# aikiriao/LINNE

Measured on NVIDIA B200. Metric: encode+decode MSamples/s over the -m 0..7 sweep, higher is better.
Workload: dtype int32+f64

## Files before the change

linne_b200/csrc/lnb_analyze_v3.cuh:

```cuda
#pragma once
#include "lnb_common.cuh"
#include "lnb_encode_core.cuh"

#define LNB_A3_THREADS  256
#define LNB_A3_WARPS    8
#define LNB_A3_MAX_NA   10240
#define LNB_A3_FRONT    160
#define LNB_A3_BACK     176
#define LNB_A3_PART     24
#define LNB_A3_ITEMS    64
#define LNB_A3_MIRROR   (LNB_MAX_PARAMS + 8)

__host__ __device__ inline uint32_t lnb_a3_array_doubles(uint32_t na_max)
{
    if (na_max < 4096u) na_max = 4096u;
    return LNB_A3_FRONT + na_max / 8u * 9u + LNB_A3_BACK;
}
__host__ __device__ inline size_t lnb_a3_smem_doubles(uint32_t na_max)
{
    return (size_t)2 * lnb_a3_array_doubles(na_max)
         + (size_t)LNB_MAX_LEVELS * LNB_MAX_PARAMS
         + (size_t)LNB_MAX_LEVELS * 256
         + (size_t)LNB_A3_ITEMS * LNB_A3_PART
         + (size_t)3 * LNB_A3_MIRROR
         + 128;
}

struct LnbA3Ctx {
    double *A, *B;
    double *cand, *acorr, *part, *lev0, *misc;
    uint32_t na, ng;
};

struct LnbA3Team {
    uint32_t tid, nthr, warp, nwarps, bar;
    __device__ __forceinline__ void sync() const
    {
        if (bar == 0u) __syncthreads();
        else asm volatile("bar.sync %0, %1;" :: "r"(bar), "r"(nthr) : "memory");
    }
};

__device__ __forceinline__ void lnb_a3_window(const LnbA3Ctx &cx, const LnbA3Team &tm, uint32_t m, double scale)
{
    const uint32_t mg = m >> 3;
    for (uint32_t G = tm.tid; G < cx.ng; G += tm.nthr) {
        const uint32_t pos0 = (G % mg) * 8u;
        const double *src = cx.A + G * 9u;
        double *dst = cx.B + G * 9u;
        const uint32_t back0 = m - 1u - pos0;
        const double a0 = (double)pos0, b0 = (double)back0;
        if (pos0 + 7u <= back0 - 7u || pos0 >= back0) {
            const bool rising = pos0 < back0;
#pragma unroll
            for (uint32_t e = 0; e < 8u; e++) {
                const double a = a0 + (double)e, b = b0 - (double)e;
                const double w = rising ? __dmul_rn(__dmul_rn(scale, a), b) : __dmul_rn(__dmul_rn(scale, b), a);
                dst[e] = __dmul_rn(src[e], w);
            }
        } else {
#pragma unroll
            for (uint32_t e = 0; e < 8u; e++) {
                const double a = a0 + (double)e, b = b0 - (double)e;
                const double q = (a < b) ? a : b, r = (a < b) ? b : a;
                dst[e] = __dmul_rn(src[e], __dmul_rn(__dmul_rn(scale, q), r));
            }
        }
    }
}

template <int L, bool MASK>
__device__ __forceinline__ void lnb_a3_tile(const double *Bg, uint32_t qoff, int32_t lim, double (&acc)[L])
{
    double s[8], wv[L + 7];
#pragma unroll
    for (int o = 0; o < 8; o++) s[o] = Bg[o];
#pragma unroll
    for (int t = 0; t < L + 7; t++) {
        const double v = (!MASK || t < lim) ? Bg[qoff + t + (t >> 3)] : 0.0;
        wv[t] = v;
    }
#pragma unroll
    for (int o = 0; o < 8; o++)
#pragma unroll
        for (int k = 0; k < L; k++) acc[k] = fma(s[o], wv[o + k], acc[k]);
}

template <int L>
__device__ __forceinline__ void lnb_a3_autocorr_item(const LnbA3Ctx &cx, uint32_t u, uint32_t q, uint32_t m, bool last_unit,
                                                     uint32_t g_lo, uint32_t g_hi, double *out )
{
    const uint32_t lane = threadIdx.x & 31u;
    const uint32_t mg = m >> 3;
    double acc[L];
#pragma unroll
    for (int k = 0; k < L; k++) acc[k] = 0.0;
    const double *Bu = cx.B + (size_t)u * mg * 9u;
    const uint32_t qoff = 18u * q;
    for (uint32_t g0 = g_lo; g0 < g_hi; g0 += 32u) {
        const uint32_t g = g0 + lane;
        const bool active = g < g_hi;
        const uint32_t gg = active ? g : g_lo;
        const int32_t lim = (int32_t)m - (int32_t)(8u * gg + 16u * q);
        const bool need_mask = !last_unit && lim < L + 7;
        if (__any_sync(0xffffffffu, need_mask)) {
            double tmp[L];
#pragma unroll
            for (int k = 0; k < L; k++) tmp[k] = 0.0;
            lnb_a3_tile<L, true>(Bu + gg * 9u, qoff, last_unit ? (int32_t)(L + 7) : lim, tmp);
            if (active) {
#pragma unroll
                for (int k = 0; k < L; k++) acc[k] += tmp[k];
            }
        } else if (active) {
            lnb_a3_tile<L, false>(Bu + gg * 9u, qoff, 0, acc);
        }
    }
    constexpr int N = (L >= 16) ? 16 : (L >= 8) ? 8 : (L >= 4) ? 4 : 2;
    constexpr int LOGN = (N == 16) ? 4 : (N == 8) ? 3 : (N == 4) ? 2 : 1;
    {
        int cnt = N;
#pragma unroll
        for (int off = 16; off > 0; off >>= 1) {
            if (cnt > 1) {
                const bool upper = (lane & (uint32_t)off) != 0u;
                const int half = cnt / 2;
#pragma unroll
                for (int k = 0; k < N / 2; k++) {
                    if (k < half) {
                        const double send = upper ? acc[k] : acc[k + half];
                        const double keep = upper ? acc[k + half] : acc[k];
                        acc[k] = keep + __shfl_xor_sync(0xffffffffu, send, off);
                    }
                }
                cnt = half;
            } else {
                acc[0] += __shfl_xor_sync(0xffffffffu, acc[0], off);
            }
        }
        if ((lane & ((1u << (5 - LOGN)) - 1u)) == 0u) out[lane >> (5 - LOGN)] = acc[0];
    }
    if (L > N) {
        double v = acc[L - 1];
#pragma unroll
        for (int off = 16; off > 0; off >>= 1) v += __shfl_xor_sync(0xffffffffu, v, off);
        if (lane == 0) out[L - 1] = v;
    }
}

__device__ void lnb_a3_autocorr(const LnbA3Ctx &cx, const LnbA3Team &tm, uint32_t U, uint32_t p, double *acorr_lvl)
{
    const uint32_t m = cx.na / U, mg = m >> 3;
    const uint32_t nq = (p >= 16u) ? p / 16u : 1u;
    const uint32_t tasks = U * nq;
    uint32_t S = 1u;
    if ((tasks % tm.nwarps) != 0u && tasks < 4u * tm.nwarps) S = (3u * tm.nwarps + tasks - 1u) / tasks;
    if (tasks * S > LNB_A3_ITEMS) S = LNB_A3_ITEMS / tasks;
    const uint32_t items = tasks * S;
    const uint32_t per = (mg + S - 1u) / S;
    for (uint32_t wi = tm.warp; wi < items; wi += tm.nwarps) {
        const uint32_t task = wi / S, split = wi % S;
        const uint32_t u = task / nq, q = task % nq;
        const uint32_t g_lo = split * per, g_hi = (g_lo + per < mg) ? g_lo + per : mg;
        const bool last_unit = (u + 1u == U);
        double *out = (S == 1u) ? acorr_lvl + u * (p + 1u) + 16u * q : cx.part + wi * LNB_A3_PART;
        if (p >= 16u) {
            if (q + 1u < nq) lnb_a3_autocorr_item<16>(cx, u, q, m, last_unit, g_lo, g_hi, out);
            else             lnb_a3_autocorr_item<17>(cx, u, q, m, last_unit, g_lo, g_hi, out);
        } else if (p == 8u)  lnb_a3_autocorr_item<9>(cx, u, q, m, last_unit, g_lo, g_hi, out);
        else if (p == 4u)    lnb_a3_autocorr_item<5>(cx, u, q, m, last_unit, g_lo, g_hi, out);
        else if (p == 2u)    lnb_a3_autocorr_item<3>(cx, u, q, m, last_unit, g_lo, g_hi, out);
        else                 lnb_a3_autocorr_item<2>(cx, u, q, m, last_unit, g_lo, g_hi, out);
    }
    if (S > 1u) {
        tm.sync();
        const uint32_t L_last = (p >= 16u) ? 17u : p + 1u;
        for (uint32_t i = tm.tid; i < tasks * 17u; i += tm.nthr) {
            const uint32_t task = i / 17u, k = i % 17u;
            const uint32_t u = task / nq, q = task % nq;
            const uint32_t Lq = (q + 1u == nq) ? L_last : 16u;
            if (k >= Lq) continue;
            double v = 0.0;
            for (uint32_t sp = 0; sp < S; sp++) v += cx.part[(task * S + sp) * LNB_A3_PART + k];
            acorr_lvl[u * (p + 1u) + 16u * q + k] = v;
        }
    }
}

__device__ __forceinline__ double lnb_a3_rcp(double x)
{
    float seed;
    asm("rcp.approx.ftz.f32 %0, %1;" : "=f"(seed) : "f"(__double2float_rn(x)));
    double y = (double)seed;
    y = fma(y, fma(-x, y, 1.0), y);
    y = fma(y, fma(-x, y, 1.0), y);
    y = fma(y, fma(-x, y, 1.0), y);
    return y;
}

__device__ void lnb_a3_levinson_warp(const double *r_in, uint32_t p, double lambda, double *scr, double *out_w)
{
    const uint32_t lane = threadIdx.x & 31u;
    const double r0 = __dmul_rn(r_in[0], __dadd_rn(1.0, lambda));
    if (fabs(r0) < (double)FLT_EPSILON) {
        for (uint32_t i = lane; i < p; i += 32u) out_w[i] = 0.0;
        return;
    }
    double *cur = scr, *nxt = scr + LNB_A3_MIRROR, *gam = scr + 2 * LNB_A3_MIRROR;
    double B[5];
#pragma unroll
    for (int s = 0; s < 5; s++) {
        const uint32_t i = lane + 32u * (uint32_t)s;
        const double ri = (i <= p) ? r_in[i] : 0.0;
        B[s] = (i == 0u) ? r0 : ri;
        if (i < LNB_A3_MIRROR) { cur[i] = ri; nxt[i] = 0.0; }
    }
    __syncwarp();
    double rinv = lnb_a3_rcp(r0);
    for (uint32_t m = 1; m <= p; m++) {
        const double gamma = -cur[1] * rinv;
        if (lane == 0) gam[m] = gamma;
        const uint32_t cnt = p - m;
        const uint32_t ns = (cnt >> 5) + 1u;
#pragma unroll
        for (int s = 0; s < 5; s++) {
            if ((uint32_t)s < ns) {
                const uint32_t i = lane + 32u * (uint32_t)s;
                if (i <= cnt) {
                    const double fs = cur[i + 1u];
                    const double b = B[s];
                    B[s] = fma(gamma, fs, b);
                    nxt[i] = fma(gamma, b, fs);
                }
            }
        }
        const double err = __shfl_sync(0xffffffffu, B[0], 0);
        rinv = lnb_a3_rcp(err);
        __syncwarp();
        double *t = cur; cur = nxt; nxt = t;
    }
    double a[5];
#pragma unroll
    for (int s = 0; s < 5; s++) {
        const uint32_t i = lane + 32u * (uint32_t)s;
        a[s] = (i == 0u) ? 1.0 : 0.0;
        if (i < LNB_A3_MIRROR) { cur[i] = a[s]; nxt[i] = a[s]; }
    }
    __syncwarp();
    for (uint32_t m = 1; m <= p; m++) {
        const double g = gam[m];
        const uint32_t ns = (m >> 5) + 1u;
#pragma unroll
        for (int s = 0; s < 5; s++) {
            if ((uint32_t)s < ns) {
                const uint32_t i = lane + 32u * (uint32_t)s;
                if (i >= 1u && i <= m) {
                    const double v = (i == m) ? g : fma(g, cur[m - i], a[s]);
                    a[s] = v;
                    nxt[i] = v;
                }
            }
        }
        __syncwarp();
        double *t = cur; cur = nxt; nxt = t;
    }
#pragma unroll
    for (int s = 0; s < 5; s++) {
        const uint32_t i = lane + 32u * (uint32_t)s;
        if (i >= 1u && i <= p) out_w[p - i] = a[s];
    }
    __syncwarp();
}

__device__ __forceinline__ void lnb_a3_fir8(const double *base, const double *w, const double (&prev)[8], double (&next)[8],
                                            double (&acc)[8])
{
#pragma unroll
    for (int k = 0; k < 8; k++) next[k] = base[7 + k + ((7 + k) >> 3)];
#pragma unroll
    for (int jj = 0; jj < 8; jj++) {
        const double wj = w[jj];
#pragma unroll
        for (int o = 0; o < 8; o++) {
            const int t = jj + o;
            acc[o] = fma(wj, (t < 7) ? prev[t + 1] : next[t - 7], acc[o]);
        }
    }
}

template <int MODE, int PS>
__device__ __forceinline__ double lnb_a3_fir(const LnbA3Ctx &cx, const LnbA3Team &tm, const double *X, double *Y, uint32_t p,
                                             uint32_t m, const double *cand_lvl)
{
    const uint32_t mg = m >> 3;
    double loss = 0.0;
    for (uint32_t G = tm.tid; G < cx.ng; G += tm.nthr) {
        const uint32_t u = G / mg;
        const double *w = cand_lvl + u * p;
        const double *Xg = X + G * 9u;
        double acc[8];
#pragma unroll
        for (int o = 0; o < 8; o++) acc[o] = (MODE == 0) ? Xg[o] : 0.0;
        if (PS == 0) {
            const double *base = Xg - (p >> 3) * 9u;
            double P[8], Q[8];
#pragma unroll
            for (int k = 0; k < 7; k++) P[k + 1] = base[k];
            uint32_t j0 = 0;
            for (; j0 + 16u <= p; j0 += 16u) {
                lnb_a3_fir8(base, w + j0, P, Q, acc);
                base += 9;
                lnb_a3_fir8(base, w + j0 + 8u, Q, P, acc);
                base += 9;
            }
            if (j0 < p) lnb_a3_fir8(base, w + j0, P, Q, acc);
        } else {
            double xw[PS + 7];
#pragma unroll
            for (int t = 0; t < PS + 7; t++) xw[t] = (t < PS) ? Xg[t - 1 - PS] : Xg[t - PS];
#pragma unroll
            for (int jj = 0; jj < PS; jj++) {
                const double wj = w[jj];
#pragma unroll
                for (int o = 0; o < 8; o++) acc[o] = fma(wj, xw[jj + o], acc[o]);
            }
        }
        if (MODE == 0) {
#pragma unroll
            for (int o = 0; o < 8; o++) if (!(G == 0u && o == 0)) loss += fabs(acc[o]);
        } else {
            double *Yg = Y + G * 9u;
#pragma unroll
            for (int o = 0; o < 8; o++) {
                const double y = Xg[o] + acc[o];
                Yg[o] = y;
                loss += fabs(y);
            }
        }
    }
    return loss;
}

template <int MODE>
__device__ double lnb_a3_fir_any(const LnbA3Ctx &cx, const LnbA3Team &tm, const double *X, double *Y, uint32_t p, uint32_t m,
                                 const double *cand_lvl)
{
    if (p >= 8u) return lnb_a3_fir<MODE, 0>(cx, tm, X, Y, p, m, cand_lvl);
    if (p == 4u) return lnb_a3_fir<MODE, 4>(cx, tm, X, Y, p, m, cand_lvl);
    if (p == 2u) return lnb_a3_fir<MODE, 2>(cx, tm, X, Y, p, m, cand_lvl);
    return lnb_a3_fir<MODE, 1>(cx, tm, X, Y, p, m, cand_lvl);
}

__device__ double lnb_a3_team_sum(const LnbA3Team &tm, double v, double *scratch )
{
#pragma unroll
    for (int off = 16; off > 0; off >>= 1) v += __shfl_xor_sync(0xffffffffu, v, off);
    tm.sync();
    if ((tm.tid & 31u) == 0) scratch[tm.warp] = v;
    tm.sync();
    double s = 0.0;
    for (uint32_t w = 0; w < tm.nwarps; w++) s += scratch[w];
    tm.sync();
    return s;
}
__device__ double lnb_a3_block_sum(double v, double *scratch)
{
    const LnbA3Team all = { threadIdx.x, LNB_A3_THREADS, threadIdx.x >> 5, LNB_A3_WARPS, 0u };
    return lnb_a3_team_sum(all, v, scratch);
}

__device__ void lnb_a3_level_losses(const LnbA3Ctx &cx, const LnbA3Team &tm, uint32_t P, uint32_t lv_first, uint32_t nlev)
{
    double *parts = cx.misc + 32;
    for (uint32_t lv = lv_first; lv < nlev; lv++) {
        const uint32_t U = 1u << lv, p = P / U;
        double v = lnb_a3_fir_any<0>(cx, tm, cx.A, (double *)0, p, cx.na / U, cx.cand + lv * LNB_MAX_PARAMS);
#pragma unroll
        for (int off = 16; off > 0; off >>= 1) v += __shfl_xor_sync(0xffffffffu, v, off);
        if ((tm.tid & 31u) == 0u) parts[tm.warp * LNB_MAX_LEVELS + lv] = v;
    }
    tm.sync();
    if (tm.tid >= lv_first && tm.tid < nlev) {
        double sum = 0.0;
        for (uint32_t w = 0; w < tm.nwarps; w++) sum += parts[w * LNB_MAX_LEVELS + tm.tid];
        cx.misc[tm.tid] = sum / (double)cx.na;
    }
}

__device__ void lnb_a3_solve_levels(const LnbA3Ctx &cx, const LnbA3Team &tm, uint32_t P, uint32_t lv_first, uint32_t nlev,
                                    double lambda, double *scratch)
{
    uint32_t thread_tasks = 0, warp_tasks = 0;
    for (uint32_t lv = lv_first; lv < nlev; lv++) { if ((P >> lv) <= 16u) thread_tasks += 1u << lv; else warp_tasks += 1u << lv; }
    for (uint32_t t = tm.tid; t < thread_tasks; t += tm.nthr) {
        uint32_t rest = t;
        for (uint32_t lv = lv_first; lv < nlev; lv++) {
            const uint32_t U = 1u << lv, p = P / U;
            if (p > 16u) continue;
            if (rest < U) {
                double r[17], a[18], coef[16];
                const double *src = cx.acorr + lv * 256 + rest * (p + 1u);
                for (uint32_t k = 0; k <= p; k++) r[k] = src[k];
                r[0] = __dmul_rn(r[0], __dadd_rn(1.0, lambda));
                lnb_levinson(r, p, a, coef, (double *)0);
                double *dst = cx.cand + lv * LNB_MAX_PARAMS + rest * p;
                for (uint32_t j = 0; j < p; j++) dst[j] = coef[p - 1u - j];
                break;
            }
            rest -= U;
        }
    }
    for (uint32_t t = tm.warp; t < warp_tasks; t += tm.nwarps) {
        uint32_t rest = t;
        for (uint32_t lv = lv_first; lv < nlev; lv++) {
            const uint32_t U = 1u << lv, p = P / U;
            if (p <= 16u) continue;
            if (rest < U) {
                lnb_a3_levinson_warp(cx.acorr + lv * 256 + rest * (p + 1u), p, lambda,
                                     scratch + tm.warp * 3 * LNB_A3_MIRROR, cx.cand + lv * LNB_MAX_PARAMS + rest * p);
                break;
            }
            rest -= U;
        }
    }
}

__device__ void lnb_a3_generic(const LnbEncodeBatch &b, uint32_t s, uint32_t bc, uint32_t blk_i, uint32_t na,
                               double lambda, uint32_t na_max, double *smem)
{
    const uint32_t c = threadIdx.x, warp = c >> 5;
    const uint32_t arr = lnb_a3_array_doubles(na_max);
    double *A = smem, *B = smem + arr;
    double *cand = smem + 2u * arr, *acorr = cand + LNB_MAX_LEVELS * LNB_MAX_PARAMS;
    double *misc = acorr + LNB_MAX_LEVELS * 256 + LNB_A3_ITEMS * LNB_A3_PART + 3 * LNB_A3_MIRROR;
    {
        const int32_t *src = b.work + (size_t)bc * b.cfg.work_stride;
        const double norm = ldexp(1.0, -(int)(b.cfg.bits_per_sample - 1u));
        for (uint32_t i = c; i < na; i += LNB_A3_THREADS) A[i] = (double)src[i] * norm;
    }
    __syncthreads();
    double final_loss = 0.0;
    for (uint32_t l = 0; l < b.cfg.num_layers; l++) {
        const uint32_t P = b.cfg.layer_params[l];
        for (uint32_t lv = 0; lv < LNB_MAX_LEVELS; lv++) {
            if (!lnb_level_valid(lv, P, na)) continue;
            const uint32_t U = 1u << lv, p = P / U, m = na / U;
            const double scale = b.welch[(size_t)blk_i * LNB_MAX_LEVELS + lv];
            for (uint32_t i = c; i < na; i += LNB_A3_THREADS)
                B[i] = lnb_mul_rn(A[i], lnb_welch_weight(scale, i % m, m));
            __syncthreads();
            for (uint32_t cell = c; cell < U * (p + 1u); cell += LNB_A3_THREADS) {
                const uint32_t lag = cell % (p + 1u);
                const double *xs = B + (size_t)(cell / (p + 1u)) * m;
                double sum = 0.0;
                for (uint32_t i = 0; i + lag < m; i++) sum = lnb_mac(xs[i], xs[i + lag], sum);
                acorr[lv * 256u + cell] = sum;
            }
            __syncthreads();
        }
        {
            uint32_t task = c, wt = warp;
            for (uint32_t lv = 0; lv < LNB_MAX_LEVELS; lv++) {
                if (!lnb_level_valid(lv, P, na)) continue;
                const uint32_t U = 1u << lv, p = P / U, m = na / U;
                if (p <= 16u) {
                    if (task < U) {
                        double r[17], a[18], coef[16];
                        const double *src = acorr + lv * 256u + task * (p + 1u);
                        for (uint32_t k = 0; k <= p; k++) r[k] = src[k];
                        r[0] = __dmul_rn(r[0], __dadd_rn(1.0, lambda));
                        if (m < p) { for (uint32_t k = 0; k < p; k++) coef[k] = 0.0; }
                        else lnb_levinson(r, p, a, coef, (double *)0);
                        double *dst = cand + lv * LNB_MAX_PARAMS + task * p;
                        for (uint32_t j = 0; j < p; j++) dst[j] = coef[p - 1u - j];
                        task = 0xFFFFFFFFu;
                    } else if (task != 0xFFFFFFFFu) task -= U;
                } else {
                    if (wt < U) {
                        double *dst = cand + lv * LNB_MAX_PARAMS + wt * p;
                        if (m < p) { for (uint32_t j = c & 31u; j < p; j += 32u) dst[j] = 0.0; }
                        else lnb_a3_levinson_warp(acorr + lv * 256u + wt * (p + 1u), p, lambda, B + warp * 3 * LNB_A3_MIRROR, dst);
                        wt = 0xFFFFFFFFu;
                    } else if (wt != 0xFFFFFFFFu) wt -= U;
                }
            }
        }
        __syncthreads();
        uint32_t best = 0;
        {
            double best_loss = (double)FLT_MAX;
            for (uint32_t lv = 0; lv < LNB_MAX_LEVELS; lv++) {
                if (!lnb_level_valid(lv, P, na)) continue;
                const uint32_t U = 1u << lv, p = P / U, m = na / U;
                double part = 0.0;
                for (uint32_t t = c; t < na; t += LNB_A3_THREADS)
                    if (t) part += fabs(lnb_residual_at(A, t, m, p, cand + lv * LNB_MAX_PARAMS, A[t]));
                const double loss = lnb_a3_block_sum(part, misc + 16) / (double)na;
                if (loss < best_loss) { best_loss = loss; best = lv; }
            }
        }
        if (c == 0) b.chosen_log2u[(size_t)s * LNB_MAX_LAYERS + l] = (uint8_t)best;
        {
            double *dst = b.chosen_w + ((size_t)s * LNB_MAX_LAYERS + l) * LNB_MAX_PARAMS;
            for (uint32_t k = c; k < P; k += LNB_A3_THREADS) dst[k] = cand[best * LNB_MAX_PARAMS + k];
        }
        {
            const uint32_t U = 1u << best, p = P / U, m = na / U;
            double part = 0.0;
            for (uint32_t t = c; t < na; t += LNB_A3_THREADS) {
                const double v = (t == 0u) ? A[0] : A[t] + lnb_residual_at(A, t, m, p, cand + best * LNB_MAX_PARAMS, 0.0);
                B[t] = v;
                part += fabs(v);
            }
            final_loss = lnb_a3_block_sum(part, misc + 16);
        }
        __syncthreads();
        double *t = A; A = B; B = t;
    }
    const uint32_t chunks_per_slot = (b.cfg.work_stride + 63u) / 64u, nch = (na + 63u) / 64u;
    for (uint32_t i = c; i < nch; i += LNB_A3_THREADS) b.final_sum[(size_t)s * chunks_per_slot + i] = (i == 0) ? final_loss : 0.0;
}

__global__ void __launch_bounds__(LNB_A3_THREADS, 1) lnb_analyze_v3_kernel(LnbEncodeBatch b, uint32_t na_max)
{
    extern __shared__ __align__(16) double lnb_a3_smem[];
    const uint32_t s = blockIdx.x, c = threadIdx.x;
    const uint32_t bc = s / b.cfg.num_lambdas, lam = s % b.cfg.num_lambdas;
    const uint32_t blk_i = bc / b.cfg.num_channels;
    const LnbBlockDesc blk = b.blocks[blk_i];
    if (blk.type != LNB_BLOCK_COMPRESSED || !(blk.status & (LNB_ENC_FLAG_FAST | LNB_ENC_FLAG_GENERIC))) return;
    if (!(blk.status & LNB_ENC_FLAG_FAST)) {
        lnb_a3_generic(b, s, bc, blk_i, blk.na, b.cfg.lambdas[lam], na_max, lnb_a3_smem);
        return;
    }

    const uint32_t arr = lnb_a3_array_doubles(na_max);
    LnbA3Ctx cx;
    cx.na = blk.na; cx.ng = blk.na >> 3;
    cx.A = lnb_a3_smem + LNB_A3_FRONT;
    cx.B = lnb_a3_smem + arr + LNB_A3_FRONT;
    cx.cand = lnb_a3_smem + 2u * arr;
    cx.acorr = cx.cand + LNB_MAX_LEVELS * LNB_MAX_PARAMS;
    cx.part = cx.acorr + LNB_MAX_LEVELS * 256;
    cx.lev0 = cx.part + LNB_A3_ITEMS * LNB_A3_PART;
    cx.misc = cx.lev0 + 3 * LNB_A3_MIRROR;
    const uint32_t na = cx.na;
    const double lambda = b.cfg.lambdas[lam];

    {
        const uint32_t data = cx.ng * 9u;
        for (uint32_t i = c; i < LNB_A3_FRONT; i += LNB_A3_THREADS) { lnb_a3_smem[i] = 0.0; lnb_a3_smem[arr + i] = 0.0; }
        for (uint32_t i = LNB_A3_FRONT + data + c; i < arr; i += LNB_A3_THREADS) { lnb_a3_smem[i] = 0.0; lnb_a3_smem[arr + i] = 0.0; }
        const int32_t *src = b.work + (size_t)bc * b.cfg.work_stride;
        const double norm = ldexp(1.0, -(int)(b.cfg.bits_per_sample - 1u));
        for (uint32_t G = c; G < cx.ng; G += LNB_A3_THREADS) {
            const int4 v0 = *(const int4 *)(src + 8u * G), v1 = *(const int4 *)(src + 8u * G + 4u);
            double *dst = cx.A + G * 9u;
            dst[0] = (double)v0.x * norm; dst[1] = (double)v0.y * norm; dst[2] = (double)v0.z * norm; dst[3] = (double)v0.w * norm;
            dst[4] = (double)v1.x * norm; dst[5] = (double)v1.y * norm; dst[6] = (double)v1.z * norm; dst[7] = (double)v1.w * norm;
            dst[8] = 0.0;
            cx.B[G * 9u + 8u] = 0.0;
        }
    }
    __syncthreads();

    double final_loss = 0.0;
    for (uint32_t l = 0; l < b.cfg.num_layers; l++) {
        const uint32_t P = b.cfg.layer_params[l];
        uint32_t nlev = 0;
        while (nlev < LNB_MAX_LEVELS && (1u << nlev) <= P) nlev++;

        const LnbA3Team all = { c, LNB_A3_THREADS, c >> 5, LNB_A3_WARPS, 0u };
        const bool split = (P >= 32u) && nlev >= 2u;
        const double *welch = b.welch + (size_t)blk_i * LNB_MAX_LEVELS;

        if (split) {
            lnb_a3_window(cx, all, na, welch[0]);
            __syncthreads();
            lnb_a3_autocorr(cx, all, 1u, P, cx.acorr);
            __syncthreads();
            if ((c >> 5) == LNB_A3_WARPS - 1u) {
                lnb_a3_levinson_warp(cx.acorr, P, lambda, cx.lev0, cx.cand);
            } else {
                const LnbA3Team rest = { c, LNB_A3_THREADS - 32u, c >> 5, LNB_A3_WARPS - 1u, 1u };
                for (uint32_t lv = 1; lv < nlev; lv++) {
                    const uint32_t U = 1u << lv, p = P / U, m = na / U;
                    lnb_a3_window(cx, rest, m, welch[lv]);
                    rest.sync();
                    lnb_a3_autocorr(cx, rest, U, p, cx.acorr + lv * 256);
                    rest.sync();
                }
                lnb_a3_solve_levels(cx, rest, P, 1u, nlev, lambda, cx.B);
                rest.sync();
                lnb_a3_level_losses(cx, rest, P, 1u, nlev);
            }
            __syncthreads();
            lnb_a3_level_losses(cx, all, P, 0u, 1u);
        } else {
            for (uint32_t lv = 0; lv < nlev; lv++) {
                const uint32_t U = 1u << lv, p = P / U, m = na / U;
                lnb_a3_window(cx, all, m, welch[lv]);
                __syncthreads();
                lnb_a3_autocorr(cx, all, U, p, cx.acorr + lv * 256);
                __syncthreads();
            }
            lnb_a3_solve_levels(cx, all, P, 0u, nlev, lambda, cx.B);
            __syncthreads();
            lnb_a3_level_losses(cx, all, P, 0u, nlev);
        }
        __syncthreads();
        uint32_t best = 0;
        {
            double best_loss = (double)FLT_MAX;
            for (uint32_t lv = 0; lv < nlev; lv++)
                if (cx.misc[lv] < best_loss) { best_loss = cx.misc[lv]; best = lv; }
        }
        if (c == 0) b.chosen_log2u[(size_t)s * LNB_MAX_LAYERS + l] = (uint8_t)best;
        {
            double *dst = b.chosen_w + ((size_t)s * LNB_MAX_LAYERS + l) * LNB_MAX_PARAMS;
            const double *src = cx.cand + best * LNB_MAX_PARAMS;
            for (uint32_t k = c; k < P; k += LNB_A3_THREADS) dst[k] = src[k];
        }

        {
            const uint32_t U = 1u << best, p = P / U;
            const double part = lnb_a3_fir_any<1>(cx, all, cx.A, cx.B, p, na / U, cx.cand + best * LNB_MAX_PARAMS);
            final_loss = lnb_a3_block_sum(part, cx.misc + 16);
        }
        __syncthreads();
        double *t = cx.A; cx.A = cx.B; cx.B = t;
    }
    {
        const uint32_t chunks_per_slot = (b.cfg.work_stride + 63u) / 64u, nch = (na + 63u) / 64u;
        for (uint32_t i = c; i < nch; i += LNB_A3_THREADS) b.final_sum[(size_t)s * chunks_per_slot + i] = (i == 0) ? final_loss : 0.0;
    }
}
```

linne_b200/csrc/lnb_shim_cuda.cu:

```cuda
#include <cuda_runtime.h>
#include <stdio.h>
#include <stdlib.h>
#include <sched.h>
#include <string.h>

#include "lnb_shim.h"
#include "lnb_pipeline.cuh"
#include "lnb_analyze_v3.cuh"
#include "lnb_pack_v2.cuh"
#include "lnb_front_v2.cuh"
#include "lnb_synth_v2.cuh"
#include "lnb_crc_v2.cuh"
#include "lnb_entropy_v3.cuh"
#include "lnb_refine_v2.cuh"
#include "lnb_scan_v2.cuh"
#include "lnb_stream_v2.cuh"
#include "lnb_hop.cuh"
#include "lnb_window.cuh"

#define LNB_MAX_STAGES 32
#define LNB_MAX_PENDING 8192
#define LNB_MAX_TIMELINE 2048

struct LnbDevice {
// ... 171 lines not shown
    }
    uint32_t synth_max_n() const { return LNB_SY_MAX_N; }
    void synth_cooperative(const LnbDecodeBatch &b)
    {
        const uint32_t items = b.num_blocks * b.cfg.num_channels;
        const uint32_t n_max = line_samples(b, LNB_SY_MAX_N);
        const size_t smem = (size_t)LNB_SY_WARPS * n_max * sizeof(int32_t);
        const int slot = begin_stage("synth_v2");
        lnb_synth_v2_kernel<<<(items + LNB_SY_WARPS - 1) / LNB_SY_WARPS, LNB_SY_THREADS, smem, dev->stream>>>(b, n_max);
        end_stage(slot);
    }
    int begin_stage(const char *name, cudaStream_t on = nullptr)
    {
        if (!dev->profiling) return -1;
        if (dev->num_pending >= LNB_MAX_PENDING) {
            cudaStreamSynchronize(dev->stream);
            if (dev->aux_created) cudaStreamSynchronize(dev->aux_stream);
            drain_profile(dev);
        }
        const int slot = dev->num_pending++;
        dev->pending_stage[slot] = stage_index(dev, name);
        cudaEventRecord(dev->ev_begin[slot], on ? on : dev->stream);
        return slot;
    }
    void end_stage(int slot, cudaStream_t on = nullptr)
    {
        if (slot >= 0) cudaEventRecord(dev->ev_end[slot], on ? on : dev->stream);
        dev->launches++;
        cudaError_t e = cudaGetLastError();
        if (e != cudaSuccess && dev->last_error == cudaSuccess) dev->last_error = e;
    }
    void scan_cooperative(const LnbEncodeBatch &b)
    {
        const int slot = begin_stage("scan_v2");
        lnb_scan_v2_kernel<<<1, LNB_SC_THREADS, 0, dev->stream>>>(b);
        end_stage(slot);
    }
    void refine_cooperative(const LnbEncodeBatch &b, uint32_t chunks_per_slot)
    {
        uint32_t na_max = b.cfg.block_size;
        uint32_t max_p = 0;
        for (uint32_t l = 0; l < b.cfg.num_layers; l++) if (b.cfg.layer_params[l] > max_p) max_p = b.cfg.layer_params[l];
        const uint32_t tri = max_p * (max_p + 1u) / 2u;
        if (b.af_iterations && na_max < tri) na_max = tri;
        na_max = (na_max + 7u) & ~7u;
        const bool global_xy = b.refine_xy != nullptr;
        const size_t smem = (global_xy ? 0u : (size_t)2 * (na_max + LNB_RF_HIST) * sizeof(double)) + sizeof(LnbRefineSmem);
        const int slot = begin_stage("refine_v2");
        lnb_refine_v2_kernel<<<b.num_blocks * b.cfg.num_channels, LNB_RF_THREADS, smem, dev->stream>>>(
            b, na_max, b.af_iterations, b.enable_learning, b.train_scratch, chunks_per_slot, global_xy ? b.refine_xy : nullptr);
        end_stage(slot);
    }
    void prepare_cooperative(const LnbEncodeBatch &b)
    {
        const int slot = begin_stage("prepare_v2");
        lnb_prepare_v2_kernel<<<b.num_blocks, LNB_FR_THREADS, 0, dev->stream>>>(b);
        end_stage(slot);
    }
    void predict_plan_cooperative(const LnbEncodeBatch &b)
    {
        uint32_t n_max = b.cfg.block_size < LNB_FR_MAX_N ? b.cfg.block_size : LNB_FR_MAX_N;
        n_max = (n_max + 3u) & ~3u;
        const size_t smem = (size_t)2 * n_max * sizeof(int32_t) + sizeof(LnbPlanSmem);
        const int slot = begin_stage("predict_plan_v2");
        lnb_predict_plan_v2_kernel<<<b.num_blocks * b.cfg.num_channels, LNB_FR_THREADS, smem, dev->stream>>>(b, n_max);
        end_stage(slot);
    }
    void pack_cooperative(const LnbEncodeBatch &b, uint32_t out_capacity)
    {
        size_t bytes = 64 + LNB_BLOCK_HEADER_SIZE + (size_t)b.cfg.block_size * b.cfg.num_channels * ((b.cfg.bits_per_sample + 7u) / 8u);
        bytes += bytes / 8;
        if (bytes > 220u * 1024u) bytes = 220u * 1024u;
        const uint32_t img_words = (uint32_t)((bytes + 3) / 4);
        const int slot = begin_stage("pack_v2");
        lnb_pack_v2_kernel<<<b.num_blocks, LNB_PK_THREADS, (size_t)img_words * 4, dev->stream>>>(b, out_capacity, img_words);
        end_stage(slot);
    }
    void analyze_cooperative(const LnbEncodeBatch &b)
    {
        const uint32_t S = b.num_blocks * b.cfg.num_channels * b.cfg.num_lambdas;
        uint32_t na_max = b.cfg.block_size < LNB_A3_MAX_NA ? b.cfg.block_size : LNB_A3_MAX_NA;
        na_max = (na_max + 7u) & ~7u;
        const size_t smem = lnb_a3_smem_doubles(na_max) * sizeof(double);
        const int slot = begin_stage("analyze_v3");
        lnb_analyze_v3_kernel<<<S, LNB_A3_THREADS, smem, dev->stream>>>(b, na_max);
        end_stage(slot);
    }
    template <class F> void run(const char *name, uint32_t n, const F &f)
    {
        if (n == 0) return;
        const uint32_t threads = 128;
        const uint32_t grid = (n + threads - 1) / threads;
        int slot = -1;
        if (dev->profiling) {
            if (dev->num_pending >= LNB_MAX_PENDING) { cudaStreamSynchronize(dev->stream); drain_profile(dev); }
            slot = dev->num_pending++;
            dev->pending_stage[slot] = stage_index(dev, name);
            cudaEventRecord(dev->ev_begin[slot], dev->stream);
        }
        lnb_items_kernel<F><<<grid, threads, 0, dev->stream>>>(n, f);
        if (slot >= 0) cudaEventRecord(dev->ev_end[slot], dev->stream);
        dev->launches++;
        cudaError_t e = cudaGetLastError();
        if (e != cudaSuccess && dev->last_error == cudaSuccess) dev->last_error = e;
    }
};

#include <mutex>
static std::mutex g_kernel_cfg_lock;
static unsigned char g_kernel_cfg_done[64];

template <class K> static cudaError_t lnb_optin_smem(K kernel, int optin_bytes)
{
    cudaFuncAttributes at;
    cudaError_t e = cudaFuncGetAttributes(&at, kernel);
    if (e != cudaSuccess) return e;
    const int dyn = optin_bytes - (int)at.sharedSizeBytes;
    return cudaFuncSetAttribute(kernel, cudaFuncAttributeMaxDynamicSharedMemorySize, dyn > 0 ? dyn : 0);
}
static int lnb_configure_kernels(int ordinal)
{
    std::lock_guard<std::mutex> guard(g_kernel_cfg_lock);
    if (ordinal >= 0 && ordinal < 64 && g_kernel_cfg_done[ordinal]) return 0;
    int optin = 0;
    if (cudaDeviceGetAttribute(&optin, cudaDevAttrMaxSharedMemoryPerBlockOptin, ordinal) != cudaSuccess) return 1;
    cudaError_t e = cudaSuccess;
    if (e == cudaSuccess) e = lnb_optin_smem(lnb_stream_v2_kernel<true>, optin);
    if (e == cudaSuccess) e = lnb_optin_smem(lnb_stream_v2_kernel<false>, optin);
    if (e == cudaSuccess) e = lnb_optin_smem(lnb_tp_synth_kernel<32, 2, 0>, optin);
    if (e == cudaSuccess) e = lnb_optin_smem(lnb_tp_synth_kernel<8, 64, 4>, optin);
    if (e == cudaSuccess) e = lnb_optin_smem(lnb_tp_synth_kernel<16, 128, 4>, optin);
    if (e == cudaSuccess) e = lnb_optin_smem(lnb_synth_v2_kernel, optin);
    if (e == cudaSuccess) e = lnb_optin_smem(lnb_refine_v2_kernel, optin);
    if (e == cudaSuccess) e = lnb_optin_smem(lnb_predict_plan_v2_kernel, optin);
    if (e == cudaSuccess) e = lnb_optin_smem(lnb_pack_v2_kernel, optin);
    if (e == cudaSuccess) e = lnb_optin_smem(lnb_analyze_v3_kernel, optin);
    if (e != cudaSuccess) {
        fprintf(stderr, "linne_b200: cannot configure kernels on device %d: %s\n", ordinal, cudaGetErrorString(e));
        cudaGetLastError();
        return 1;
    }
    if (ordinal >= 0 && ordinal < 64) g_kernel_cfg_done[ordinal] = 1;
    return 0;
}

extern "C" {

const char *lnb_shim_backend(void) { return "cuda-sm_100a"; }
int lnb_shim_device_count(void) { int n = 0; if (cudaGetDeviceCount(&n) != cudaSuccess) { cudaGetLastError(); return 0; } return n; }
int lnb_shim_set_device(int ordinal) { if (cudaSetDevice(ordinal) != cudaSuccess) { cudaGetLastError(); return 1; } return 0; }
int lnb_shim_device_ordinal(const LnbDevice *dev) { return dev->ordinal; }
int lnb_shim_current_device(void) { int d = -1; if (cudaGetDevice(&d) != cudaSuccess) { cudaGetLastError(); return -1; } return d; }
uint32_t lnb_shim_fast_max_na(void) { return LNB_A3_MAX_NA; }
uint32_t lnb_shim_coop_max_n(void) { return LNB_FR_MAX_N; }
uint32_t lnb_shim_refine_max_na(void) { return LNB_RF_MAX_NA; }
uint32_t lnb_shim_refine_hist(void) { return LNB_RF_HIST; }
uint32_t lnb_shim_fused_max_n(void) { return LNB_DS_MAX_N; }
int lnb_shim_tput_supported(const LnbStreamCfg *cfg)
{
    return lnb_tput_shape(cfg) != 0 && cfg->block_size <= LNB_DS_MAX_N && (cfg->block_size & 1023u) == 0u
        && cfg->bits_per_sample <= 31u && !(cfg->ms && (cfg->num_channels & 1u));
}

int lnb_shim_open(LnbDevice **out, int device_ordinal)
{
    int count = 0;
    {
        static int once = 0;
        if (!__atomic_exchange_n(&once, 1, __ATOMIC_ACQ_REL)) setenv("CUDA_DEVICE_MAX_CONNECTIONS", "32", 0);
    }
    if (cudaGetDeviceCount(&count) != cudaSuccess || count <= 0) return 1;
    if (device_ordinal >= 0) {
        if (device_ordinal >= count || cudaSetDevice(device_ordinal) != cudaSuccess) return 2;
    }
    LnbDevice *dev = (LnbDevice *)calloc(1, sizeof(LnbDevice));
    if (!dev) return 3;
    cudaGetDevice(&dev->ordinal);
    if (lnb_configure_kernels(dev->ordinal)) { free(dev); return 7; }
    if (cudaStreamCreateWithFlags(&dev->stream, cudaStreamNonBlocking) != cudaSuccess) { free(dev); return 4; }
    dev->owns_stream = 1;
    dev->cost_rank = -1;
    {
        const char *mode = getenv("LINNE_B200_SYNC");
        if (mode && mode[0] == 'b' && cudaEventCreateWithFlags(&dev->sync_event, cudaEventBlockingSync | cudaEventDisableTiming) == cudaSuccess)
            dev->blocking_sync = 1;
        if (mode && mode[0] == 'y') dev->yield_sync = 1;
    }

    const LnbHostTables *ht = lnb_tables_get();
    const size_t sz_lut = sizeof(ht->huff_lut), sz_code = sizeof(ht->huff_code), sz_len = 256,
                 sz_thr = sizeof(ht->k2_threshold), sz_crc = sizeof(ht->crc_table);
    const size_t total = sz_lut + sz_code + sz_thr + sz_crc + sz_len + 64;
    uint8_t *mem = NULL;
    if (cudaMalloc((void **)&mem, total) != cudaSuccess) { cudaStreamDestroy(dev->stream); free(dev); return 5; }
    size_t off = 0;
    cudaMemcpy(mem + off, ht->k2_threshold, sz_thr, cudaMemcpyHostToDevice); dev->tables.k2_threshold = (const double *)(mem + off); off += sz_thr;
    cudaMemcpy(mem + off, ht->huff_code, sz_code, cudaMemcpyHostToDevice);   dev->tables.huff_code = (const uint32_t *)(mem + off); off += sz_code;
    cudaMemcpy(mem + off, ht->huff_lut, sz_lut, cudaMemcpyHostToDevice);     dev->tables.huff_lut = (const uint16_t *)(mem + off); off += sz_lut;
    cudaMemcpy(mem + off, ht->crc_table, sz_crc, cudaMemcpyHostToDevice);    dev->tables.crc_table = (const uint16_t *)(mem + off); off += sz_crc;
    cudaMemcpy(mem + off, ht->huff_len, sz_len, cudaMemcpyHostToDevice);     dev->tables.huff_len = (const uint8_t *)(mem + off); off += sz_len;
    dev->table_mem = mem;
    if (cudaDeviceSynchronize() != cudaSuccess) { cudaFree(mem); cudaStreamDestroy(dev->stream); free(dev); return 6; }
    *out = dev;
    return 0;
}

void lnb_shim_close(LnbDevice *dev)
{
    bind_device(dev);
    if (!dev) return;
    cudaStreamSynchronize(dev->stream);
    if (dev->events_created)
        for (int i = 0; i < LNB_MAX_PENDING; i++) { cudaEventDestroy(dev->ev_begin[i]); cudaEventDestroy(dev->ev_end[i]); }
    cudaFree(dev->table_mem);
    if (dev->blocking_sync) cudaEventDestroy(dev->sync_event);
    if (dev->aux_created) { cudaStreamDestroy(dev->aux_stream); cudaEventDestroy(dev->ev_fork); cudaEventDestroy(dev->ev_join); }
    if (dev->owns_stream) cudaStreamDestroy(dev->stream);
    free(dev);
}

const LnbDevTables *lnb_shim_tables(const LnbDevice *dev) { return &dev->tables; }

void lnb_shim_use_stream(LnbDevice *dev, void *cuda_stream)
{
    bind_device(dev);
    if (dev->owns_stream) { cudaStreamSynchronize(dev->stream); cudaStreamDestroy(dev->stream); dev->owns_stream = 0; }
    dev->stream = (cudaStream_t)cuda_stream;
}

void lnb_shim_set_cost_rank(LnbDevice *dev, int cost_rank)
{
    bind_device(dev);
    if (!dev->owns_stream || dev->cost_rank == cost_rank) return;
    { const char *e = getenv("LINNE_B200_STREAM_PRIORITY"); if (e && *e == '0') return; }
    int least = 0, greatest = 0;
    if (cudaDeviceGetStreamPriorityRange(&least, &greatest) != cudaSuccess) { cudaGetLastError(); return; }
    int span = least - greatest;
    if (span <= 0) return;
    if (cost_rank < 0) cost_rank = 0;
    if (cost_rank > 7) cost_rank = 7;
    const int prio = least - (cost_rank * span + 3) / 7;
    cudaStream_t s;
    if (cudaStreamCreateWithPriority(&s, cudaStreamNonBlocking, prio) != cudaSuccess) { cudaGetLastError(); return; }
    cudaStreamSynchronize(dev->stream);
    cudaStreamDestroy(dev->stream);
    dev->stream = s;
    dev->cost_rank = cost_rank;
    if (dev->aux_created) {
        cudaStreamSynchronize(dev->aux_stream);
        cudaStreamDestroy(dev->aux_stream); cudaEventDestroy(dev->ev_fork); cudaEventDestroy(dev->ev_join);
        dev->aux_created = 0;
    }
}

void *lnb_shim_alloc(LnbDevice *dev, size_t bytes)
{
    void *p = NULL;
    bind_device(dev);
    if (bytes == 0) bytes = 16;
    if (cudaMalloc(&p, bytes) != cudaSuccess) { cudaGetLastError(); return NULL; }
    return p;
}
void lnb_shim_free(LnbDevice *dev, void *ptr) { bind_device(dev); if (ptr) cudaFree(ptr); }
void *lnb_shim_alloc_pinned(size_t bytes)
{
    void *p = NULL;
    if (cudaMallocHost(&p, bytes ? bytes : 16) != cudaSuccess) { cudaGetLastError(); return NULL; }
    return p;
}
void lnb_shim_free_pinned(void *ptr) { if (ptr) cudaFreeHost(ptr); }

static int note(LnbDevice *dev, cudaError_t e)
{
    if (e != cudaSuccess && dev->last_error == cudaSuccess) dev->last_error = e;
    return e == cudaSuccess ? 0 : 1;
}
int lnb_shim_h2d(LnbDevice *dev, void *dst, const void *src, size_t bytes)
{
    bind_device(dev);
    return bytes ? note(dev, cudaMemcpyAsync(dst, src, bytes, cudaMemcpyHostToDevice, dev->stream)) : 0;
}
int lnb_shim_d2d(LnbDevice *dev, void *dst, const void *src, size_t bytes)
{
    bind_device(dev);
    return bytes ? note(dev, cudaMemcpyAsync(dst, src, bytes, cudaMemcpyDeviceToDevice, dev->stream)) : 0;
}
int lnb_shim_d2h(LnbDevice *dev, void *dst, const void *src, size_t bytes)
{
    bind_device(dev);
    return bytes ? note(dev, cudaMemcpyAsync(dst, src, bytes, cudaMemcpyDeviceToHost, dev->stream)) : 0;
}
int lnb_shim_memset(LnbDevice *dev, void *dst, int value, size_t bytes)
{
    bind_device(dev);
    return bytes ? note(dev, cudaMemsetAsync(dst, value, bytes, dev->stream)) : 0;
}
int lnb_shim_sync(LnbDevice *dev)
{
    bind_device(dev);
    cudaError_t e;
    if (dev->blocking_sync) {
        e = cudaEventRecord(dev->sync_event, dev->stream);
        if (e == cudaSuccess) e = cudaEventSynchronize(dev->sync_event);
    } else if (dev->yield_sync) {
        while ((e = cudaStreamQuery(dev->stream)) == cudaErrorNotReady) sched_yield();
    } else {
// ... 219 lines not shown
```

Baseline: 1634.

## Process two FIR groups per thread and share level-0 loss work dynamically

The FIR loss/forward loop now handles two 8-sample groups per thread per iteration. When both groups use the same coefficient set, the weight loads are shared, which raises instruction-level parallelism and reuse. The level-0 loss in the split path is broken into per-warp units claimed through an atomic counter, so the Levinson warp can start on loss work as soon as it finishes instead of waiting for the final block-wide pass. Optional clock64-based phase timing instrumentation is added behind a compile flag. The changes raise register pressure, and the unit-claiming scheme adds an atomic and an extra block sync.

```diff
diff --git a/linne_b200/csrc/lnb_analyze_v3.cuh b/linne_b200/csrc/lnb_analyze_v3.cuh
--- a/linne_b200/csrc/lnb_analyze_v3.cuh
+++ b/linne_b200/csrc/lnb_analyze_v3.cuh
@@ -32,14 +32,70 @@
     uint32_t na, ng;
 };
 
+enum {
+    LNB_A3_PH_LOAD = 0, LNB_A3_PH_WINDOW, LNB_A3_PH_ACORR,
+    LNB_A3_PH_LEV0 = LNB_A3_PH_ACORR + LNB_MAX_LEVELS,
+    LNB_A3_PH_SOLVE, LNB_A3_PH_LOSS, LNB_A3_PH_FORWARD, LNB_A3_PH_WAIT,
+    LNB_A3_PH_CTAS, LNB_A3_NPH
+};
+#ifdef LNB_A3_TIMING
+__device__ unsigned long long lnb_a3_clk[LNB_A3_NPH];
+__shared__ long long lnb_a3_tmark[LNB_A3_WARPS];
+__shared__ int lnb_a3_tphase[LNB_A3_WARPS];
+__device__ __forceinline__ void lnb_a3_phase(int ph)
+{
+    if ((threadIdx.x & 31u) == 0u) {
+        const uint32_t w = threadIdx.x >> 5;
+        const long long now = clock64();
+        if (lnb_a3_tphase[w] >= 0) atomicAdd(&lnb_a3_clk[lnb_a3_tphase[w]], (unsigned long long)(now - lnb_a3_tmark[w]));
+        lnb_a3_tmark[w] = now;
+        lnb_a3_tphase[w] = ph;
+    }
+}
+__device__ __forceinline__ void lnb_a3_wait_end()
+{
+    if ((threadIdx.x & 31u) == 0u) {
+        const uint32_t w = threadIdx.x >> 5;
+        const long long now = clock64();
+        if (lnb_a3_tphase[w] >= 0) atomicAdd(&lnb_a3_clk[LNB_A3_PH_WAIT], (unsigned long long)(now - lnb_a3_tmark[w]));
+        lnb_a3_tmark[w] = now;
+    }
+}
+__device__ __forceinline__ void lnb_a3_clock_start(bool fast)
+{
+    if ((threadIdx.x & 31u) == 0u) {
+        lnb_a3_tphase[threadIdx.x >> 5] = fast ? (int)LNB_A3_PH_LOAD : -1;
+        lnb_a3_tmark[threadIdx.x >> 5] = clock64();
+    }
+    if (fast && threadIdx.x == 0u) atomicAdd(&lnb_a3_clk[LNB_A3_PH_CTAS], 1ull);
+}
+#define LNB_A3_CLOCK_START(fast) lnb_a3_clock_start(fast)
+#define LNB_A3_PHASE(ph)      lnb_a3_phase(ph)
+#define LNB_A3_WAIT_BEGIN()   lnb_a3_phase(lnb_a3_tphase[threadIdx.x >> 5])
+#define LNB_A3_WAIT_END()     lnb_a3_wait_end()
+#else
+#define LNB_A3_CLOCK_START(fast) ((void)0)
+#define LNB_A3_PHASE(ph)      ((void)0)
+#define LNB_A3_WAIT_BEGIN()   ((void)0)
+#define LNB_A3_WAIT_END()     ((void)0)
+#endif
+
 struct LnbA3Team {
     uint32_t tid, nthr, warp, nwarps, bar;
     __device__ __forceinline__ void sync() const
     {
+        LNB_A3_WAIT_BEGIN();
         if (bar == 0u) __syncthreads();
         else asm volatile("bar.sync %0, %1;" :: "r"(bar), "r"(nthr) : "memory");
+        LNB_A3_WAIT_END();
     }
 };
+__device__ __forceinline__ void lnb_a3_sync_all()
+{
+    LNB_A3_WAIT_BEGIN();
+    __syncthreads();
+    LNB_A3_WAIT_END();
+}
 
 __device__ __forceinline__ void lnb_a3_window(const LnbA3Ctx &cx, const LnbA3Team &tm, uint32_t m, double scale)
 {
@@ -272,48 +328,104 @@
     __syncwarp();
 }
 
-__device__ __forceinline__ void lnb_a3_fir8(const double *base, const double *w, const double (&prev)[8], double (&next)[8],
-                                            double (&acc)[8])
-{
-#pragma unroll
-    for (int k = 0; k < 8; k++) next[k] = base[7 + k + ((7 + k) >> 3)];
+template <int NG, bool SW>
+__device__ __forceinline__ void lnb_a3_fir8(const double *const (&base)[NG], const double *const (&w)[NG], const double (&prev)[NG][8],
+                                            double (&next)[NG][8], double (&acc)[NG][8])
+{
+#pragma unroll
+    for (int g = 0; g < NG; g++)
+#pragma unroll
+        for (int k = 0; k < 8; k++) next[g][k] = base[g][7 + k + ((7 + k) >> 3)];
 #pragma unroll
     for (int jj = 0; jj < 8; jj++) {
-        const double wj = w[jj];
+        double wj[NG];
+#pragma unroll
+        for (int g = 0; g < NG; g++) wj[g] = (SW && g > 0) ? wj[0] : w[g][jj];
+#pragma unroll
+        for (int g = 0; g < NG; g++)
+#pragma unroll
+            for (int o = 0; o < 8; o++) {
+                const int t = jj + o;
+                acc[g][o] = fma(wj[g], (t < 7) ? prev[g][t + 1] : next[g][t - 7], acc[g][o]);
+            }
+    }
+}
+
+template <int NG, bool SW>
+__device__ __forceinline__ void lnb_a3_fir_slide(const double *const (&Xg)[NG], const double *const (&wg)[NG], uint32_t p,
+                                                 double (&acc)[NG][8])
+{
+    const double *base[NG], *w[NG];
+    double P[NG][8], Q[NG][8];
+#pragma unroll
+    for (int g = 0; g < NG; g++) {
+        base[g] = Xg[g] - (p >> 3) * 9u;
+        w[g] = wg[g];
+#pragma unroll
+        for (int k = 0; k < 7; k++) P[g][k + 1] = base[g][k];
+    }
+    uint32_t j0 = 0;
+    for (; j0 + 16u <= p; j0 += 16u) {
+        lnb_a3_fir8<NG, SW>(base, w, P, Q, acc);
+#pragma unroll
+        for (int g = 0; g < NG; g++) { base[g] += 9; w[g] += 8; }
+        lnb_a3_fir8<NG, SW>(base, w, Q, P, acc);
+#pragma unroll
+        for (int g = 0; g < NG; g++) { base[g] += 9; w[g] += 8; }
+    }
+    if (j0 < p) lnb_a3_fir8<NG, SW>(base, w, P, Q, acc);
+}
+
+template <int MODE>
+__device__ __forceinline__ void lnb_a3_fir_out(const double *Xg, double *Y, uint32_t G, const double (&acc)[8], double &loss)
+{
+    if (MODE == 0) {
+#pragma unroll
+        for (int o = 0; o < 8; o++) if (!(G == 0u && o == 0)) loss += fabs(acc[o]);
+    } else {
+        double *Yg = Y + G * 9u;
 #pragma unroll
         for (int o = 0; o < 8; o++) {
-            const int t = jj + o;
-            acc[o] = fma(wj, (t < 7) ? prev[t + 1] : next[t - 7], acc[o]);
-        }
-    }
-}
-
+            const double y = Xg[o] + acc[o];
+            Yg[o] = y;
+            loss += fabs(y);
+        }
+    }
+}
 template <int MODE, int PS>
 __device__ __forceinline__ double lnb_a3_fir(const LnbA3Ctx &cx, const LnbA3Team &tm, const double *X, double *Y, uint32_t p,
                                              uint32_t m, const double *cand_lvl)
 {
     const uint32_t mg = m >> 3;
     double loss = 0.0;
-    for (uint32_t G = tm.tid; G < cx.ng; G += tm.nthr) {
+    uint32_t G = tm.tid;
+    if (PS == 0) {
+        for (; G + tm.nthr < cx.ng; G += 2u * tm.nthr) {
+            const uint32_t G1 = G + tm.nthr, u0 = G / mg, u1 = G1 / mg;
+            const double *const Xg[2] = { X + G * 9u, X + G1 * 9u };
+            const double *const w[2] = { cand_lvl + u0 * p, cand_lvl + u1 * p };
+            double acc[2][8];
+#pragma unroll
+            for (int g = 0; g < 2; g++)
+#pragma unroll
+                for (int o = 0; o < 8; o++) acc[g][o] = (MODE == 0) ? Xg[g][o] : 0.0;
+            if (u0 == u1) lnb_a3_fir_slide<2, true>(Xg, w, p, acc);
+            else          lnb_a3_fir_slide<2, false>(Xg, w, p, acc);
+            lnb_a3_fir_out<MODE>(Xg[0], Y, G, acc[0], loss);
+            lnb_a3_fir_out<MODE>(Xg[1], Y, G1, acc[1], loss);
+        }
+    }
+    for (; G < cx.ng; G += tm.nthr) {
         const uint32_t u = G / mg;
         const double *w = cand_lvl + u * p;
         const double *Xg = X + G * 9u;
-        double acc[8];
-#pragma unroll
-        for (int o = 0; o < 8; o++) acc[o] = (MODE == 0) ? Xg[o] : 0.0;
+        double acc[1][8];
+#pragma unroll
+        for (int o = 0; o < 8; o++) acc[0][o] = (MODE == 0) ? Xg[o] : 0.0;
         if (PS == 0) {
-            const double *base = Xg - (p >> 3) * 9u;
-            double P[8], Q[8];
-#pragma unroll
-            for (int k = 0; k < 7; k++) P[k + 1] = base[k];
-            uint32_t j0 = 0;
-            for (; j0 + 16u <= p; j0 += 16u) {
-                lnb_a3_fir8(base, w + j0, P, Q, acc);
-                base += 9;
-                lnb_a3_fir8(base, w + j0 + 8u, Q, P, acc);
-                base += 9;
-            }
-            if (j0 < p) lnb_a3_fir8(base, w + j0, P, Q, acc);
+            const double *const Xs[1] = { Xg };
+            const double *const ws[1] = { w };
+            lnb_a3_fir_slide<1, true>(Xs, ws, p, acc);
         } else {
             double xw[PS + 7];
 #pragma unroll
@@ -322,21 +434,10 @@
             for (int jj = 0; jj < PS; jj++) {
                 const double wj = w[jj];
 #pragma unroll
-                for (int o = 0; o < 8; o++) acc[o] = fma(wj, xw[jj + o], acc[o]);
-            }
-        }
-        if (MODE == 0) {
-#pragma unroll
-            for (int o = 0; o < 8; o++) if (!(G == 0u && o == 0)) loss += fabs(acc[o]);
-        } else {
-            double *Yg = Y + G * 9u;
-#pragma unroll
-            for (int o = 0; o < 8; o++) {
-                const double y = Xg[o] + acc[o];
-                Yg[o] = y;
-                loss += fabs(y);
-            }
-        }
+                for (int o = 0; o < 8; o++) acc[0][o] = fma(wj, xw[jj + o], acc[0][o]);
+            }
+        }
+        lnb_a3_fir_out<MODE>(Xg, Y, G, acc[0], loss);
     }
     return loss;
 }
@@ -384,6 +485,23 @@
         double sum = 0.0;
         for (uint32_t w = 0; w < tm.nwarps; w++) sum += parts[w * LNB_MAX_LEVELS + tm.tid];
         cx.misc[tm.tid] = sum / (double)cx.na;
+    }
+}
+
+__device__ void lnb_a3_level0_loss_units(const LnbA3Ctx &cx, uint32_t P, uint32_t *next_unit)
+{
+    const uint32_t lane = threadIdx.x & 31u;
+    double *parts = cx.misc + 32;
+    for (;;) {
+        uint32_t k = 0;
+        if (lane == 0u) k = atomicAdd(next_unit, 1u);
+        k = __shfl_sync(0xffffffffu, k, 0);
+        if (k >= LNB_A3_WARPS) break;
+        const LnbA3Team unit = { k * 32u + lane, LNB_A3_THREADS, k, LNB_A3_WARPS, 0u };
+        double v = lnb_a3_fir_any<0>(cx, unit, cx.A, (double *)0, P, cx.na, cx.cand);
+#pragma unroll
+        for (int off = 16; off > 0; off >>= 1) v += __shfl_xor_sync(0xffffffffu, v, off);
+        if (lane == 0u) parts[k * LNB_MAX_LEVELS] = v;
     }
 }
 
@@ -529,6 +647,7 @@
     const uint32_t blk_i = bc / b.cfg.num_channels;
     const LnbBlockDesc blk = b.blocks[blk_i];
     if (blk.type != LNB_BLOCK_COMPRESSED || !(blk.status & (LNB_ENC_FLAG_FAST | LNB_ENC_FLAG_GENERIC))) return;
+    LNB_A3_CLOCK_START((blk.status & LNB_ENC_FLAG_FAST) != 0u);
     if (!(blk.status & LNB_ENC_FLAG_FAST)) {
         lnb_a3_generic(b, s, bc, blk_i, blk.na, b.cfg.lambdas[lam], na_max, lnb_a3_smem);
         return;
@@ -562,7 +681,7 @@
             cx.B[G * 9u + 8u] = 0.0;
         }
     }
-    __syncthreads();
+    lnb_a3_sync_all();
 
     double final_loss = 0.0;
     for (uint32_t l = 0; l < b.cfg.num_layers; l++) {
@@ -575,40 +694,63 @@
         const double *welch = b.welch + (size_t)blk_i * LNB_MAX_LEVELS;
 
         if (split) {
+            uint32_t *next_unit = (uint32_t *)(cx.misc + 100);
+            if (c == 0u) *next_unit = 0u;
+            LNB_A3_PHASE(LNB_A3_PH_WINDOW);
             lnb_a3_window(cx, all, na, welch[0]);
-            __syncthreads();
+            lnb_a3_sync_all();
+            LNB_A3_PHASE(LNB_A3_PH_ACORR);
             lnb_a3_autocorr(cx, all, 1u, P, cx.acorr);
-            __syncthreads();
+            lnb_a3_sync_all();
             if ((c >> 5) == LNB_A3_WARPS - 1u) {
+                LNB_A3_PHASE(LNB_A3_PH_LEV0);
                 lnb_a3_levinson_warp(cx.acorr, P, lambda, cx.lev0, cx.cand);
+                LNB_A3_PHASE(LNB_A3_PH_LOSS);
+                lnb_a3_level0_loss_units(cx, P, next_unit);
             } else {
                 const LnbA3Team rest = { c, LNB_A3_THREADS - 32u, c >> 5, LNB_A3_WARPS - 1u, 1u };
                 for (uint32_t lv = 1; lv < nlev; lv++) {
                     const uint32_t U = 1u << lv, p = P / U, m = na / U;
+                    LNB_A3_PHASE(LNB_A3_PH_WINDOW);
                     lnb_a3_window(cx, rest, m, welch[lv]);
                     rest.sync();
+                    LNB_A3_PHASE(LNB_A3_PH_ACORR + lv);
                     lnb_a3_autocorr(cx, rest, U, p, cx.acorr + lv * 256);
                     rest.sync();
                 }
+                LNB_A3_PHASE(LNB_A3_PH_SOLVE);
                 lnb_a3_solve_levels(cx, rest, P, 1u, nlev, lambda, cx.B);
                 rest.sync();
+                LNB_A3_PHASE(LNB_A3_PH_LOSS);
                 lnb_a3_level_losses(cx, rest, P, 1u, nlev);
             }
-            __syncthreads();
-            lnb_a3_level_losses(cx, all, P, 0u, 1u);
+            lnb_a3_sync_all();
+            LNB_A3_PHASE(LNB_A3_PH_LOSS);
+            lnb_a3_level0_loss_units(cx, P, next_unit);
+            lnb_a3_sync_all();
+            if (c == 0u) {
+                double sum = 0.0;
+                for (uint32_t w = 0; w < LNB_A3_WARPS; w++) sum += cx.misc[32 + w * LNB_MAX_LEVELS];
+                cx.misc[0] = sum / (double)na;
+            }
         } else {
             for (uint32_t lv = 0; lv < nlev; lv++) {
                 const uint32_t U = 1u << lv, p = P / U, m = na / U;
+                LNB_A3_PHASE(LNB_A3_PH_WINDOW);
                 lnb_a3_window(cx, all, m, welch[lv]);
-                __syncthreads();
+                lnb_a3_sync_all();
+                LNB_A3_PHASE(LNB_A3_PH_ACORR + lv);
                 lnb_a3_autocorr(cx, all, U, p, cx.acorr + lv * 256);
-                __syncthreads();
-            }
+                lnb_a3_sync_all();
+            }
+            LNB_A3_PHASE(LNB_A3_PH_SOLVE);
             lnb_a3_solve_levels(cx, all, P, 0u, nlev, lambda, cx.B);
-            __syncthreads();
+            lnb_a3_sync_all();
+            LNB_A3_PHASE(LNB_A3_PH_LOSS);
             lnb_a3_level_losses(cx, all, P, 0u, nlev);
         }
-        __syncthreads();
+        lnb_a3_sync_all();
+        LNB_A3_PHASE(LNB_A3_PH_FORWARD);
         uint32_t best = 0;
         {
             double best_loss = (double)FLT_MAX;
@@ -627,11 +769,12 @@
             const double part = lnb_a3_fir_any<1>(cx, all, cx.A, cx.B, p, na / U, cx.cand + best * LNB_MAX_PARAMS);
             final_loss = lnb_a3_block_sum(part, cx.misc + 16);
         }
-        __syncthreads();
+        lnb_a3_sync_all();
         double *t = cx.A; cx.A = cx.B; cx.B = t;
     }
     {
         const uint32_t chunks_per_slot = (b.cfg.work_stride + 63u) / 64u, nch = (na + 63u) / 64u;
         for (uint32_t i = c; i < nch; i += LNB_A3_THREADS) b.final_sum[(size_t)s * chunks_per_slot + i] = (i == 0) ? final_loss : 0.0;
     }
-}
+    LNB_A3_PHASE(-1);
+}
diff --git a/linne_b200/csrc/lnb_shim_cuda.cu b/linne_b200/csrc/lnb_shim_cuda.cu
--- a/linne_b200/csrc/lnb_shim_cuda.cu
+++ b/linne_b200/csrc/lnb_shim_cuda.cu
@@ -347,6 +347,15 @@
 int lnb_shim_device_ordinal(const LnbDevice *dev) { return dev->ordinal; }
 int lnb_shim_current_device(void) { int d = -1; if (cudaGetDevice(&d) != cudaSuccess) { cudaGetLastError(); return -1; } return d; }
 uint32_t lnb_shim_fast_max_na(void) { return LNB_A3_MAX_NA; }
+#ifdef LNB_A3_TIMING
+int lnb_shim_a3_phase_clocks(unsigned long long *out, int n)
+{
+    unsigned long long z[LNB_A3_NPH] = {0};
+    if (n < LNB_A3_NPH || cudaDeviceSynchronize() != cudaSuccess) return 1;
+    if (cudaMemcpyFromSymbol(out, lnb_a3_clk, sizeof(z)) != cudaSuccess) return 1;
+    return cudaMemcpyToSymbol(lnb_a3_clk, z, sizeof(z)) != cudaSuccess;
+}
+#endif
 uint32_t lnb_shim_coop_max_n(void) { return LNB_FR_MAX_N; }
 uint32_t lnb_shim_refine_max_na(void) { return LNB_RF_MAX_NA; }
 uint32_t lnb_shim_refine_hist(void) { return LNB_RF_HIST; }
```

Measured after the change: 1629 (median of 6 runs). No clear change (-0.3%).
